# yeyupiaoling/VoiceprintRecognition-PaddlePaddle

Measured on AMD Instinct MI355X. Metric: utterances/sec (3 s, 16 kHz) ECAPA-TDNN fwd+AAM, higher is better.
Workload: dtype bf16; 1 GPU; BASELINE configs[1]: ECAPA-TDNN (C=512, MFA 1536, ASP, embd 192) + Kaldi Fbank 80, 3 s @ 16 kHz (T=298), 2796-class cosine head + AAMLoss, eval-mode forward, batch 256 per GPU, inputs resident in HBM, random-init weights; batch_per_gpu=256, global_batch=256, parallelism=dp1 (no collective), streams_per_gpu=2, hip_graph=True, graph_prereplays=40

## Files before the change

include/vpmi.h:

```cpp
#ifndef VPMI_H
#define VPMI_H
#include <stddef.h>
#include <stdint.h>

#ifdef __cplusplus
extern "C" {
#endif

#define VPMI_VERSION 100

typedef struct vp_ctx vp_ctx;
typedef void* vp_stream;

enum { VP_OK = 0, VP_EINVAL = -1, VP_ENOMEM = -2, VP_EHIP = -3, VP_EUNSUP = -4, VP_EWORKSPACE = -5 };
enum { VP_F32 = 0, VP_BF16 = 1,
       VP_F32X3 = 2,
       VP_HL32 = 3 };
enum { VP_PAD_NONE = 0, VP_PAD_REFLECT = 1, VP_PAD_ZERO = 2 };
enum { VP_ACT_NONE = 0, VP_ACT_RELU = 1, VP_ACT_SIGMOID = 2, VP_ACT_TANH = 3,
       VP_ACT_HARDTANH20 = 4,
       VP_ACT_SILU = 5 };

int vp_version(void);
vp_ctx* vp_create(int device);
void vp_destroy(vp_ctx* ctx);
const char* vp_last_error(vp_ctx* ctx);
int vp_set_margin_table(vp_ctx* ctx, const float* table);

typedef struct {
    int sample_rate;
    int n_mels;
    float frame_length_ms;
    float frame_shift_ms;
    float preemph;
    int remove_dc;
    float low_freq;
    float high_freq;
    float log_floor;
} vp_fbank_opts;

void vp_fbank_default_opts(vp_fbank_opts* o);
int vp_fbank_num_frames(const vp_fbank_opts* o, int n_samples);
size_t vp_fbank_workspace_bytes(const vp_fbank_opts* o, int B, int L);
int vp_fbank_cmn_f32(vp_ctx* ctx, const float* wav, const float* lens_ratio, int B, int L,
                     const vp_fbank_opts* o, float* out, void* out_bf16, void* ws, size_t ws_bytes,
                     vp_stream stream);
int vp_fbank_cmn_pcm16(vp_ctx* ctx, const int16_t* wav, float pcm_scale, const float* lens_ratio, int B, int L,
                       const vp_fbank_opts* o, float* out, void* out_bf16, void* ws, size_t ws_bytes, vp_stream stream);

int vp_fbank_cmn_ragged_f32(vp_ctx* ctx, const float* wav, const int32_t* n_samples, int B, int L, const vp_fbank_opts* o,
                            float* out, void* out_bf16, int32_t* n_frames, void* ws, size_t ws_bytes, vp_stream stream);

typedef struct {
    int sample_rate;
    int n_fft;
    int hop_length;
    int win_length;
    int n_mels;
    float f_min;
    float f_max;
    float power;
    int log_db;
    float amin;
    float ref_value;
} vp_mel_opts;

void vp_mel_default_opts(vp_mel_opts* o);
int vp_mel_num_frames(const vp_mel_opts* o, int n_samples);
size_t vp_mel_workspace_bytes(const vp_mel_opts* o, int B, int L);
int vp_melspec_cmn_f32(vp_ctx* ctx, const float* wav, const float* lens_ratio, int B, int L,
                       const vp_mel_opts* o, float* out, void* out_bf16, void* ws, size_t ws_bytes,
                       vp_stream stream);

int vp_melspec_cmn_ragged_f32(vp_ctx* ctx, const float* wav, const int32_t* n_samples, int B, int L, const vp_mel_opts* o,
                              float* out, void* out_bf16, int32_t* n_frames, void* ws, size_t ws_bytes, vp_stream stream);

typedef struct {
    int dtype_in, dtype_out;
    int B, T_in, T_out;
    int Cin, Cout, KW, dilation, stride, pad_left, pad_mode;
    const void* x;   int ldx, xoff;
    const void* w;
    const float* bias;
    const float* rowbias;
    int act;
    const float* bn_scale;
    const float* bn_shift;
    int act2;
    void* y;         int ldy, yoff;
    void* y2;        int ldy2, y2off, ysplit;
    const void* add_in; int ld_add, add_off;
    void* aux;       int ld_aux, aux_off;
    float* psum;
    float* psumsq;
    int F_in, F_out, KF, stride_f, pad_f;
    const float* pro_scale;
    const float* pro_shift;
    const void* res; int ld_res, res_off;
    const float* gate; int gate_len, gate_nseg;
    int mfma_bf16;
} vp_conv1d_desc;

int vp_conv1d_tiles_m(int B, int T_out);
int vp_conv1d_nseg(int T_out);
int vp_conv1d_fwd(vp_ctx* ctx, const vp_conv1d_desc* d, vp_stream stream);
enum { VP_CONV_K128 = 0,
       VP_CONV_K256_TWO_STAGE = 1,
       VP_CONV_K256_RING = 2,
       VP_CONV_K128X256_RING = 3 };
int vp_conv1d_plan(const vp_conv1d_desc* d, int* kernel, int* tile_n, int* tiles_m, int* tiles_n, int* group_m, int* launches);
int vp_conv256_select(int schedule);

int vp_moments_finalize(vp_ctx* ctx, const float* psum, const float* psumsq, const float* shift,
                        int B, int T, int C, float eps, int want_std, float* stats, vp_stream stream);
int vp_moments_finalize_affine(vp_ctx* ctx, const float* psum, const float* psumsq, const float* scale, const float* shift,
                               int B, int T, int C, float eps, int want_std, float* stats, vp_stream stream);

int vp_dense_f32(vp_ctx* ctx, const float* a, int lda, const float* w, int w_is_kn, const float* bias,
                 int M, int N, int K, int act, float* out, int ldo, vp_stream stream);

int vp_cast_f32_bf16(vp_ctx* ctx, const float* x, void* y, long long n, vp_stream stream);


int vp_se_scale_residual(vp_ctx* ctx, int dtype, const void* x, int ldx, int xoff, const float* s,
                         const void* res, int ldr, int roff, void* out, int ldo, int ooff,
                         int B, int T, int C, vp_stream stream);
int vp_se_scale_residual_shadow(vp_ctx* ctx, const float* x, int ldx, int xoff, const float* s, const float* res, int ldr, int roff,
                                float* out, int ldo, int ooff, void* shadow, int ld_shadow, int shadow_off, int B, int T, int C,
                                vp_stream stream);

int vp_asp_softmax_stats(vp_ctx* ctx, int dtype, const float* logits, const void* x, int ldx, int xoff,
                         int B, int T, int C, float eps, float* pooled, vp_stream stream);

#define VP_MAX_SE_BLOCKS 8
#define VP_MAX_RES2 15

typedef struct {
    const void* w;
    const float* bias;
    const float* bn_scale;
    const float* bn_shift;
    int cin, cout, kw, dil;
    const void* w_hl;
} vp_tdnn_layer;

typedef struct {
    vp_tdnn_layer tdnn1;
    vp_tdnn_layer res2[VP_MAX_RES2];
    vp_tdnn_layer tdnn2;
    const float* se_w1;
    const float* se_b1;
    const float* se_w2;
    const float* se_b2;
} vp_se_res2_block;

typedef struct {
    vp_tdnn_layer tdnn;
    const float* w_ctx;
    const void* conv_w;
    const float* conv_b;
    int C, att;
} vp_asp_weights;

typedef struct {
    int dtype;
    int feat_dim, embd_dim, n_blocks, res2_scale, se_ch;
    vp_tdnn_layer block0;
    vp_se_res2_block blk[VP_MAX_SE_BLOCKS];
    vp_tdnn_layer mfa;
    vp_asp_weights asp;
    const float* fc_w;
    const float* fc_b;
} vp_ecapa_weights;

int vp_res2_chain_fwd(vp_ctx* ctx, const vp_tdnn_layer* layers, int nconv, const void* t1, void* r2, int B, int T, int C,
                      int width, vp_stream stream);
int vp_asp_fused_fwd(vp_ctx* ctx, const void* h, const void* w, const float* bias, const void* x, int ldx, const float* center,
                     int ldc, int B, int T, int C, int att, float eps, float* pooled, vp_stream stream);
int vp_se_gate_fwd(vp_ctx* ctx, const float* psum, const float* shift, int B, int T, int C, int H, const float* w1, const float* b1,
                   const float* w2, const float* b2, float* out, vp_stream stream);
int vp_asp_utt_fwd(vp_ctx* ctx, const void* x, int ldx, const vp_tdnn_layer* tdnn, const float* rowbias, const void* conv_w,
                   const float* conv_b, int B, int T, int C, int att, float eps, float* pooled, vp_stream stream);

int vp_res2_chain_x3_fwd(vp_ctx* ctx, const vp_tdnn_layer* layers, int nconv, const void* t1, void* r2, int B, int T, int C,
                         int width, vp_stream stream);
int vp_res2_chain_x3_plan(int T, int nconv, int dil, int* nsplit, int* tseg, int* tp, int* lds_bytes);
int vp_ecapa_x3_fast_path(const vp_ecapa_weights* w, int B, int T);
int vp_asp_fused_x3_fwd(vp_ctx* ctx, const void* h, const float* w, const float* bias, const void* x, int ldx, const float* center,
                        int ldc, int B, int T, int C, int att, float eps, float* pooled, vp_stream stream);

size_t vp_ecapa_workspace_bytes(const vp_ecapa_weights* w, int B, int T);
int vp_ecapa_fwd(vp_ctx* ctx, const vp_ecapa_weights* w, const void* feats, int B, int T, float* emb,
                 void* ws, size_t ws_bytes, vp_stream stream);

typedef struct {
    int dtype;
    int feat_dim, embd_dim, channels;
    vp_tdnn_layer td[5];
    vp_asp_weights asp;
    const float* lin_w;
    const float* lin_b;
} vp_tdnn_weights;

size_t vp_tdnn_workspace_bytes(const vp_tdnn_weights* w, int B, int T);
int vp_tdnn_fwd(vp_ctx* ctx, const vp_tdnn_weights* w, const void* feats, int B, int T, float* emb,
                void* ws, size_t ws_bytes, vp_stream stream);

#define VP_MAX_CAM_LAYERS 64
#define VP_MAX_CAM_BLOCKS 4

typedef struct {
    vp_tdnn_layer conv1, conv2, shortcut;
    int stride, has_shortcut;
} vp_resblock;

typedef struct {
    const float* bn1_scale;
    const float* bn1_shift;
    vp_tdnn_layer linear1;
    vp_tdnn_layer local;
    const float* ctx_w1;
    const float* ctx_b1;
    const float* ctx_w2;
    const float* ctx_b2;
} vp_cam_layer;

typedef struct {
    const float* bn_scale;
    const float* bn_shift;
    vp_tdnn_layer linear;
} vp_transit;

typedef struct {
    int dtype;
    int feat_dim, embd_dim, m_channels, init_channels, growth, bn_channels, seg_len;
    int n_blocks;
    int block_layers[VP_MAX_CAM_BLOCKS];
    const float* fcm1_w;
    const float* fcm1_b;
    const float* fcm1_scale;
    const float* fcm1_shift;
    vp_resblock res[4];
    vp_tdnn_layer fcm_conv2;
    vp_tdnn_layer tdnn;
    vp_cam_layer layers[VP_MAX_CAM_LAYERS];
    vp_transit transit[VP_MAX_CAM_BLOCKS];
    const float* out_bn_scale;
    const float* out_bn_shift;
    const float* dense_w;
    const float* dense_b;
} vp_campplus_weights;

int vp_cam_block_fwd(vp_ctx* ctx, const vp_cam_layer* layers, int n_layers, void* cat, int ld, int ch0, int B, int Tn, int seg_len,
                     int bn_channels, int growth, vp_stream stream);
int vp_resblock_c32_fwd(vp_ctx* ctx, const void* x, void* y, const vp_tdnn_layer* conv1, const vp_tdnn_layer* conv2, int B, int T, int F,
                        vp_stream stream);
int vp_conv3x3_c32_fwd(vp_ctx* ctx, const void* x, void* y, const vp_tdnn_layer* conv, const void* res, int relu,
                       const vp_tdnn_layer* shortcut, void* y2, int B, int T, int F_in, int stride_f, const void* c1_feats,
                       const float* c1_w, const float* c1_b, const float* c1_scale, const float* c1_shift, vp_stream stream);

size_t vp_campplus_workspace_bytes(const vp_campplus_weights* w, int B, int T);
int vp_campplus_fwd(vp_ctx* ctx, const vp_campplus_weights* w, const void* feats, int B, int T, float* emb,
                    void* ws, size_t ws_bytes, vp_stream stream);

int vp_spec_augment(vp_ctx* ctx, int dtype, void* feats, int B, int T, int F, const int32_t* fmask, int n_freq_masks,
                    const int32_t* tmask, int n_time_masks, int replace_with_zero, vp_stream stream);
int vp_pad_batch(vp_ctx* ctx, int dtype, const void* const* srcs, const int32_t* lens, int B, int Tmax, int F, void* out,
                 vp_stream stream);
int vp_wave_batch_f32(vp_ctx* ctx, const float* const* srcs, const int32_t* lens, const int32_t* starts, int B, int L,
                      int normalize, float target_db, const float* gain_db, float* out, int32_t* n_valid, vp_stream stream);
int vp_speed_perturb_f32(vp_ctx* ctx, const float* const* srcs, const int32_t* lens, const int32_t* new_lens,
                         float* const* dsts, int B, int max_new_len, vp_stream stream);
int vp_noise_mix_f32(vp_ctx* ctx, const float* const* srcs, const int32_t* lens, const float* const* noises,
                     const int32_t* noise_lens, const int32_t* noise_starts, const float* snr_db, float* const* dsts, int B,
                     vp_stream stream);
size_t vp_reverb_workspace_bytes(int B, int max_len, int max_rir_len);
int vp_reverb_f32(vp_ctx* ctx, const float* const* srcs, const int32_t* lens, const float* const* rirs, const int32_t* rir_lens,
                  float* const* dsts, int B, int max_len, int max_rir_len, void* ws, size_t ws_bytes, vp_stream stream);

#define VP_MAX_RSE_BLOCKS 32

typedef struct {
    vp_tdnn_layer conv1, conv2, conv3, down;
    const float* se_w1;
    const float* se_b1;
    const float* se_w2;
    const float* se_b2;
    int stride, has_down;
} vp_rse_block;

typedef struct {
    int dtype;
    int feat_dim, embd_dim, n_blocks, c1_channels;
    const float* c1_w;
    const float* c1_b;
    const float* c1_scale;
    const float* c1_shift;
    vp_rse_block blk[VP_MAX_RSE_BLOCKS];
    vp_asp_weights asp;
    const float* lin_w;
    const float* lin_b;
} vp_resnetse_weights;

int vp_pointwise_fwd(vp_ctx* ctx, const vp_conv1d_desc* d, vp_stream stream);
size_t vp_resnetse_workspace_bytes(const vp_resnetse_weights* w, int B, int T);
int vp_resnetse_fwd(vp_ctx* ctx, const vp_resnetse_weights* w, const void* feats, int B, int T, float* emb,
                    void* ws, size_t ws_bytes, vp_stream stream);

#define VP_MAX_ERE_BLOCKS 40
#define VP_MAX_ERE_SCALE 4

typedef struct { vp_tdnn_layer c1, c2; } vp_aff_weights;

typedef struct {
    vp_tdnn_layer conv1;
    vp_tdnn_layer convs[VP_MAX_ERE_SCALE];
    vp_tdnn_layer conv3;
    vp_tdnn_layer shortcut;
    vp_aff_weights fuse[VP_MAX_ERE_SCALE - 1];
    int stride, has_shortcut, use_aff, width, scale;
} vp_ere_block;

typedef struct {
    int dtype;
    int feat_dim, embd_dim, n_blocks, m_channels;
    int stage_blocks[4];
    int first_fuse;
    const float* c1_w;
    const float* c1_b;
    const float* c1_scale;
    const float* c1_shift;
    vp_ere_block blk[VP_MAX_ERE_BLOCKS];
    vp_tdnn_layer down[3];
    vp_aff_weights fuse[3];
    const float* seg_w;
    const float* seg_b;
} vp_eres2net_weights;

size_t vp_eres2net_workspace_bytes(const vp_eres2net_weights* w, int B, int T);
int vp_eres2net_fwd(vp_ctx* ctx, const vp_eres2net_weights* w, const void* feats, int B, int T, float* emb,
                    void* ws, size_t ws_bytes, vp_stream stream);

#define VP_MAX_R2N_BLOCKS 32
#define VP_MAX_R2N_SCALE 8

typedef struct {
    vp_tdnn_layer conv1;
    vp_tdnn_layer convs[VP_MAX_R2N_SCALE];
    vp_tdnn_layer conv3;
    vp_tdnn_layer down;
    int stride, has_down, stage, width, scale;
} vp_r2n_block;

typedef struct {
    int dtype;
    int feat_dim, embd_dim, n_blocks, m_channels;
    const float* c1_w;
    const float* c1_b;
    const float* c1_scale;
    const float* c1_shift;
    vp_r2n_block blk[VP_MAX_R2N_BLOCKS];
    vp_asp_weights asp;
    const float* lin_w;
    const float* lin_b;
} vp_res2net_weights;

size_t vp_res2net_workspace_bytes(const vp_res2net_weights* w, int B, int T);
int vp_res2net_fwd(vp_ctx* ctx, const vp_res2net_weights* w, const void* feats, int B, int T, float* emb,
                   void* ws, size_t ws_bytes, vp_stream stream);
int vp_res2net_stem_fwd(vp_ctx* ctx, int dtype, const void* feats, void* out, const float* w, const float* bias, const float* scale,
                        const float* shift, int B, int T, int F, int C, vp_stream stream);
int vp_avgpool3x3_fwd(vp_ctx* ctx, int dtype, const void* x, int ldx, int xoff, void* y, int ldy, int yoff, int B, int T, int F, int C,
                      int stride, vp_stream stream);
int vp_avgpool3x3_bwd_f32(vp_ctx* ctx, const float* dy, int lddy, int dyoff, float* dx, int lddx, int dxoff, int B, int T, int F, int C,
                          int stride, vp_stream stream);
int vp_maxpool3x3_fwd_f32(vp_ctx* ctx, const float* x, float* y, int B, int T, int F, int C, vp_stream stream);
int vp_maxpool3x3_bwd_f32(vp_ctx* ctx, const float* x, const float* dy, float* dx, int B, int T, int F, int C, vp_stream stream);

size_t vp_cosine_logits_workspace_bytes(int B, int D, int C);
int vp_cosine_logits_f32(vp_ctx* ctx, const float* emb, const float* W, int B, int D, int C, float* logits,
                         void* ws, size_t ws_bytes, vp_stream stream);
int vp_aam_ce_fwd(vp_ctx* ctx, const float* logits, const int64_t* labels, int B, int C, float margin, float scale,
                  float label_smoothing, int easy_margin, float* loss, float* row_loss,
                  vp_stream stream);
size_t vp_cosine_aam_workspace_bytes(int B, int D, int C);
int vp_cosine_aam_ce_fwd(vp_ctx* ctx, const float* emb, const float* W, const int64_t* labels, int B, int D,
                         int C, float margin, float scale, float label_smoothing, int easy_margin,
                         float* loss, float* logits, float* row_loss, void* ws, size_t ws_bytes,
                         vp_stream stream);

size_t vp_cosine_aam_tiled_workspace_bytes(int B, int D, int C);
int vp_cosine_aam_tiled_fwd(vp_ctx* ctx, const float* emb, const float* W, const int64_t* labels, int B, int D, int C, float margin,
                            float scale, float label_smoothing, int easy_margin, float* loss, float* row_loss, float* lse,
                            float* cinv, int* pred, void* ws, size_t ws_bytes, vp_stream stream);

size_t vp_cosine_aam_tiled_bwd_workspace_bytes(int B, int D, int C);
int vp_cosine_aam_tiled_bwd(vp_ctx* ctx, const float* emb, const float* W, const int64_t* labels, int B, int D, int C, float margin,
                            float scale, float label_smoothing, int easy_margin, float grad_scale, float* demb, float* dW, float* loss,
                            int* pred, void* ws, size_t ws_bytes, vp_stream stream);

size_t vp_cosine_aam_ce_bwd_workspace_bytes(int B, int D, int C);
int vp_cosine_aam_ce_bwd(vp_ctx* ctx, const float* emb, const float* W, const int64_t* labels, int B, int D, int C, float margin,
                         float scale, float label_smoothing, int easy_margin, float grad_scale, float* demb, float* dW,
                         float* loss, void* ws, size_t ws_bytes, vp_stream stream);

int vp_aam_ce_bwd(vp_ctx* ctx, const float* logits, const int64_t* labels, int B, int C, float margin, float scale,
                  float label_smoothing, int easy_margin, float grad_scale, float* dlogits, float* loss, float* row_loss,
                  vp_stream stream);
size_t vp_cosine_logits_bwd_workspace_bytes(int B, int D, int C);
int vp_cosine_logits_bwd(vp_ctx* ctx, const float* emb, const float* W, const float* dcos, int B, int D, int C, float* demb,
                         float* dW, void* ws, size_t ws_bytes, vp_stream stream);

enum { VP_LOSS_AAM = 0, VP_LOSS_AM = 1, VP_LOSS_ARM = 2, VP_LOSS_CE = 3, VP_LOSS_SUBCENTER = 4 };
int vp_margin_ce_fwd(vp_ctx* ctx, const float* logits, const int64_t* labels, int B, int C, int K, int kind, float margin,
                     float scale, float label_smoothing, int easy_margin, float* loss, float* row_loss, vp_stream stream);
int vp_margin_ce_bwd(vp_ctx* ctx, const float* logits, const int64_t* labels, int B, int C, int K, int kind, float margin,
                     float scale, float label_smoothing, int easy_margin, float grad_scale, float* dlogits, float* loss,
                     float* row_loss, vp_stream stream);
int vp_sphereface2(vp_ctx* ctx, const float* logits, const int64_t* labels, const float* bias, int B, int C, float margin,
                   float scale, float lanbuda, int t, int margin_type_a, float grad_scale, float* loss, float* row_loss,
                   float* dlogits, float* dbias, float* row_dbias, vp_stream stream);

size_t vp_conv1d_wgrad_workspace_bytes(const vp_conv1d_desc* d);
int vp_conv1d_wgrad_f32(vp_ctx* ctx, const vp_conv1d_desc* d, const float* dz, int lddz, float* dW, void* ws, size_t ws_bytes,
                        vp_stream stream);
int vp_conv1d_wgrad_oik_f32(vp_ctx* ctx, const vp_conv1d_desc* d, const float* dz, int lddz, float* dW, void* ws, size_t ws_bytes,
                            vp_stream stream);
int vp_conv_weight_layouts_f32(vp_ctx* ctx, const float* w, int Cout, int Cin, int KW, float* wp, float* w2, vp_stream stream);
int vp_conv2d_weight_layouts_f32(vp_ctx* ctx, const float* w, int Cout, int Cin, int KF, int KT, float* wp, float* w2, vp_stream stream);
int vp_prep_weights_bf16(vp_ctx* ctx, const void* const* w, void* const* w16, void* const* wt16, const int* rows, const int* cols,
                         const int* ld, int n, vp_stream stream);
size_t vp_col_sums_workspace_bytes(long long M, int C);
int vp_col_sums_f32(vp_ctx* ctx, const float* a, int lda, const float* b, int ldb, const float* bmean, const float* bscale,
                    long long M, int C, float* sums, void* ws, size_t ws_bytes, vp_stream stream);
int vp_bn_train_finalize(vp_ctx* ctx, const float* psum, const float* psumsq, int nparts, long long M, int C, const float* gamma,
                         const float* beta, float* running_mean, float* running_var, float momentum, float eps, float* mean,
                         float* invstd, float* scale, float* shift, vp_stream stream);
int vp_affine_rows_f32(vp_ctx* ctx, const float* z, int ldz, const float* scale, const float* shift, long long M, int C, float* y,
                       int ldy, int relu, vp_stream stream);
int vp_bn_relu_bwd_f32(vp_ctx* ctx, const float* dy, int lddy, const float* z, int ldz, const float* mean, const float* invstd,
                       const float* gamma, const float* sums, long long M, int C, int relu_mask, float* dz, int lddz,
                       vp_stream stream);
size_t vp_bn_relu_bwd_dbias_workspace_bytes(long long M, int C);
int vp_bn_relu_bwd_dbias_f32(vp_ctx* ctx, const float* dy, int lddy, const float* z, int ldz, const float* mean, const float* invstd,
                             const float* gamma, const float* sums, long long M, int C, int relu_mask, float* dz, int lddz,
                             float* dbias, void* ws, size_t ws_bytes, vp_stream stream);
int vp_bn_relu_bwd_dbias_bf16out(vp_ctx* ctx, const float* dy, int lddy, const float* z, int ldz, const float* mean, const float* invstd,
                                 const float* gamma, const float* sums, long long M, int C, int relu_mask, void* dz, int lddz,
                                 float* dbias, void* ws, size_t ws_bytes, vp_stream stream);
int vp_conv1d_wgrad_bf16_oik(vp_ctx* ctx, const vp_conv1d_desc* d, const void* dz, int lddz, float* dW, void* ws, size_t ws_bytes,
                             vp_stream stream);
int vp_affine_rows_b16_f32(vp_ctx* ctx, const void* z, int ldz, const float* scale, const float* shift, long long M, int C, float* y,
                           int ldy, int relu, vp_stream stream);
int vp_col_sums_f32_b16(vp_ctx* ctx, const float* a, int lda, const void* b, int ldb, const float* bmean, const float* bscale, long long M,
                        int C, float* sums, void* ws, size_t ws_bytes, vp_stream stream);
int vp_bn_relu_bwd_dbias_b16(vp_ctx* ctx, const float* dy, int lddy, const void* z, int ldz, const float* mean, const float* invstd,
                             const float* gamma, const float* sums, long long M, int C, int relu_mask, void* dz, int lddz,
                             float* dbias, void* ws, size_t ws_bytes, vp_stream stream);
int vp_pack_segments_f32(vp_ctx* ctx, const void* const* srcs, const long long* offs, const long long* sizes, int n, float* dst,
                         vp_stream stream);
int vp_adam_step_f32(vp_ctx* ctx, float* param, const float* grad, float* m, float* v, long long n, float lr, float beta1, float beta2,
                     float eps, float weight_decay, int step, float grad_scale, vp_stream stream);
int vp_adamw_step_f32(vp_ctx* ctx, float* param, const float* grad, float* m, float* v, long long n, float lr, float beta1, float beta2,
                      float eps, float coeff, int step, float grad_scale, vp_stream stream);
int vp_momentum_step_f32(vp_ctx* ctx, float* param, const float* grad, float* velocity, long long n, float lr, float momentum,
                         float weight_decay, int use_nesterov, float grad_scale, vp_stream stream);

int vp_utt_sums_f32(vp_ctx* ctx, const float* a, int lda, int B, int T, int C, float* out, vp_stream stream);
int vp_time_stats_f32(vp_ctx* ctx, const float* x, int ldx, int B, int T, int C, float eps, int unbiased ,
                      float* stats, vp_stream stream);
int vp_time_stats_bwd_add_f32(vp_ctx* ctx, const float* x, int ldx, const float* stats, const float* dstats, int B, int T, int C, float eps,
                              int unbiased, const float* add, int ldadd, float* dx, int lddx, vp_stream stream);
int vp_time_stats_bwd_f32(vp_ctx* ctx, const float* x, int ldx, const float* stats, const float* dstats, int B, int T, int C, float eps,
                          int unbiased, float* dx, int lddx, vp_stream stream);
int vp_attn_stats_bwd_f32(vp_ctx* ctx, const float* e, const float* x, int ldx, const float* pooled, const float* dpooled, int B, int T,
                          int C, float eps, float* de, float* dx, int lddx, vp_stream stream);
int vp_attn_stats_bwd_de16(vp_ctx* ctx, const float* e, const float* x, int ldx, const float* pooled, const float* dpooled, int B, int T,
                           int C, float eps, void* de, float* dx, int lddx, vp_stream stream);
int vp_asp_softmax_stats_l16(vp_ctx* ctx, const void* logits_bf16, const void* x, int x_dtype, int ldx, int xoff, int B, int T, int C, float eps,
// ... 123 lines not shown
```

voiceprintrecognition-paddlepaddle_amd/csrc/res2_chain.hip:

```cpp
#include "common.h"

namespace {

constexpr int R2_W = 64;
constexpr int R2_K = 3 * R2_W;
constexpr int R2_THREADS = 512;
constexpr int R2_WAVES = R2_THREADS / 64;
constexpr int R2_ROUNDS = 3;
typedef __attribute__((address_space(3))) void* r2_lds_ptr;

struct Res2Args {
    const bf16_t* t1;
    bf16_t* r2;
    const bf16_t* w[VP_MAX_RES2];
    const float* bias[VP_MAX_RES2];
    const float* scale[VP_MAX_RES2];
    const float* shift[VP_MAX_RES2];
    int T, C, nconv, dil, TP;
    unsigned t1_bytes;
#ifdef VP_TIMING
    unsigned long long* dbg;
#endif
};

__device__ __forceinline__ int reflect_idx(int t, int T) {
    t = t < 0 ? -t : t;
    return t >= T ? 2 * (T - 1) - t : t;
}

__global__ __launch_bounds__(R2_THREADS, 1) void res2_chain_kernel(Res2Args a) {
    extern __shared__ __attribute__((aligned(16))) char smem[];
    const int act_bytes = a.TP * 128;
    char* act0 = smem;
    char* wt0 = smem + 2 * act_bytes;
    constexpr int WT_BYTES = R2_W * R2_K * 2;
#ifdef VP_TIMING
    unsigned long long stamps[32];
    int nst = 0;
    stamps[nst++] = wall_clock64();
#endif
    const int tid = threadIdx.x, lane = tid & 63;
    const int wv = __builtin_amdgcn_readfirstlane(tid >> 6);
    const int li = lane & 15, g = lane >> 4;
    const int b = blockIdx.x;
    const size_t row0 = (size_t)b * a.T;
    constexpr unsigned OOB = 0xfffffff0u;
    const __amdgpu_buffer_rsrc_t xsrd = __builtin_amdgcn_make_buffer_rsrc(const_cast<bf16_t*>(a.t1), 0, a.t1_bytes, 0x00020000);

    const int drow = lane >> 3;
    const unsigned dchunk = (unsigned)((lane & 7) ^ drow) << 4;
    auto dma_x = [&](int slice, char* dst) {
        const unsigned colb = (unsigned)slice * (R2_W * 2) + dchunk;
        for (int p = wv; p < a.TP / 8; p += R2_WAVES) {
            const int t = p * 8 + drow;
            const unsigned off = t < a.T ? (unsigned)((row0 + t) * a.C * 2) + colb : OOB;
            __builtin_amdgcn_raw_ptr_buffer_load_lds(xsrd, (r2_lds_ptr)(dst + p * 1024), 16, off, 0, 0, 0);
        }
    };
    auto dma_w = [&](int j, char* dst) {
        const __amdgpu_buffer_rsrc_t wsrd = __builtin_amdgcn_make_buffer_rsrc(const_cast<bf16_t*>(a.w[j]), 0, WT_BYTES, 0x00020000);
#pragma unroll
        for (int u = 0; u < 3; ++u) {
            const int p = wv + u * R2_WAVES;
            const int tap = p >> 3, nb = (p & 7) * 8;
            const unsigned off = (unsigned)((nb + drow) * (R2_K * 2) + tap * 128) + dchunk;
            __builtin_amdgcn_raw_ptr_buffer_load_lds(wsrd, (r2_lds_ptr)(dst + tap * 8192 + nb * 128), 16, off, 0, 0, 0);
        }
    };

    dma_x(1, act0);
    dma_w(0, wt0);
    const int ntile = a.TP / 16;
    float* prm = reinterpret_cast<float*>(wt0 + 2 * WT_BYTES);
    for (int i = tid; i < a.nconv * 192; i += R2_THREADS) {
        const int j = i / 192, k = i - j * 192, which = k >> 6, n = k & 63;
        prm[i] = which == 0 ? a.bias[j][n] : (which == 1 ? a.scale[j][n] : a.shift[j][n]);
    }
    asm volatile("s_waitcnt vmcnt(0)" ::: "memory");
    __syncthreads();
#ifdef VP_TIMING
    stamps[nst++] = wall_clock64();
#endif

    for (int j = 0; j < a.nconv; ++j) {
        char* ain = act0 + (j & 1) * act_bytes;
        char* aout = act0 + ((j + 1) & 1) * act_bytes;
        const char* wl = wt0 + (j & 1) * WT_BYTES;
        const bool has_next = j + 1 < a.nconv;
        if (has_next) {
            dma_x(j + 2, aout);
            dma_w(j + 1, wt0 + ((j + 1) & 1) * WT_BYTES);
        }
        bf16x8 wf[4][6];
#pragma unroll
        for (int ni = 0; ni < 4; ++ni) {
            const int n = ni * 16 + li;
#pragma unroll
            for (int s = 0; s < 6; ++s) {
                const int c = (s & 1) * 4 + g;
                wf[ni][s] = *reinterpret_cast<const bf16x8*>(wl + (s >> 1) * 8192 + n * 128 + ((c ^ (n & 7)) << 4));
            }
        }
        f32x4 acc[R2_ROUNDS][4];
#pragma unroll
        for (int r = 0; r < R2_ROUNDS; ++r) {
            const int mt = wv + r * R2_WAVES;
            const int t = min(mt * 16 + li, a.TP - 1);
#pragma unroll
            for (int ni = 0; ni < 4; ++ni) acc[r][ni] = f32x4{0.f, 0.f, 0.f, 0.f};
#pragma unroll
            for (int tap = 0; tap < 3; ++tap) {
                int ts = reflect_idx(t + (tap - 1) * a.dil, a.T);
                ts = min(max(ts, 0), a.TP - 1);
#pragma unroll
                for (int ks = 0; ks < 2; ++ks) {
                    const int c = ks * 4 + g;
                    const bf16x8 xf = *reinterpret_cast<const bf16x8*>(ain + ts * 128 + ((c ^ (ts & 7)) << 4));
#pragma unroll
                    for (int ni = 0; ni < 4; ++ni)
                        acc[r][ni] = __builtin_amdgcn_mfma_f32_16x16x32_bf16(wf[ni][tap * 2 + ks], xf, acc[r][ni], 0, 0, 0);
                }
            }
        }
#ifdef VP_TIMING
        if (nst < 32) stamps[nst++] = wall_clock64();
#endif
        asm volatile("s_waitcnt vmcnt(0)" ::: "memory");
        __syncthreads();
#ifdef VP_TIMING
        if (nst < 32) stamps[nst++] = wall_clock64();
#endif
        const float* pj = prm + j * 192;
#pragma unroll
        for (int r = 0; r < R2_ROUNDS; ++r) {
            const int mt = wv + r * R2_WAVES;
            if (mt < ntile) {
                const int t = mt * 16 + li;
#pragma unroll
                for (int ni = 0; ni < 4; ++ni) {
                    const int nb = ni * 16 + g * 4;
                    const float4 bb = *reinterpret_cast<const float4*>(pj + nb);
                    const float4 ss = *reinterpret_cast<const float4*>(pj + 64 + nb);
                    const float4 hh = *reinterpret_cast<const float4*>(pj + 128 + nb);
                    float v[4];
                    v[0] = fmaxf(acc[r][ni][0] + bb.x, 0.f) * ss.x + hh.x;
                    v[1] = fmaxf(acc[r][ni][1] + bb.y, 0.f) * ss.y + hh.y;
                    v[2] = fmaxf(acc[r][ni][2] + bb.z, 0.f) * ss.z + hh.z;
                    v[3] = fmaxf(acc[r][ni][3] + bb.w, 0.f) * ss.w + hh.w;
                    const int pos = t * 128 + (((nb >> 3) ^ (t & 7)) << 4) + (nb & 7) * 2;
                    bf16x4 o;
                    o[0] = (bf16_t)v[0]; o[1] = (bf16_t)v[1]; o[2] = (bf16_t)v[2]; o[3] = (bf16_t)v[3];
                    *reinterpret_cast<bf16x4*>(ain + pos) = o;
                    if (has_next) {
                        const bf16x4 xn = *reinterpret_cast<const bf16x4*>(aout + pos);
                        bf16x4 s;
                        s[0] = (bf16_t)(v[0] + (float)xn[0]); s[1] = (bf16_t)(v[1] + (float)xn[1]);
                        s[2] = (bf16_t)(v[2] + (float)xn[2]); s[3] = (bf16_t)(v[3] + (float)xn[3]);
                        *reinterpret_cast<bf16x4*>(aout + pos) = s;
                    }
                }
            }
        }
        __syncthreads();
#ifdef VP_TIMING
        if (nst < 32) stamps[nst++] = wall_clock64();
#endif
        {
            bf16_t* ybase = a.r2 + row0 * a.C + (j + 1) * R2_W;
            for (int i = tid; i < a.T * 8; i += R2_THREADS) {
                const int t = i >> 3, c = i & 7;
                const uint4 v = *reinterpret_cast<const uint4*>(ain + t * 128 + ((c ^ (t & 7)) << 4));
                *reinterpret_cast<uint4*>(ybase + (size_t)t * a.C + c * 8) = v;
            }
        }
        __syncthreads();
#ifdef VP_TIMING
        if (nst < 32) stamps[nst++] = wall_clock64();
#endif
    }
#ifdef VP_TIMING
    if (a.dbg && tid == 0)
        for (int i = 0; i < 32; ++i) a.dbg[(size_t)b * 32 + i] = i < nst ? stamps[i] : 0;
#endif
}

}

#ifdef VP_TIMING
static unsigned long long* g_res2_dbg = nullptr;
extern "C" void vp_dbg_res2_buffer(void* p) { g_res2_dbg = (unsigned long long*)p; }
#endif

int vp_res2_chain_bf16(vp_ctx* ctx, const vp_tdnn_layer* layers, int nconv, const void* t1, void* r2, int B, int T,
                       int C, int width, hipStream_t st) {
    if (width != R2_W || nconv < 1 || nconv > VP_MAX_RES2) return VP_EUNSUP;
    const int TP = (T + 15) / 16 * 16;
    const size_t smem = (size_t)2 * TP * 128 + 2 * (size_t)R2_W * R2_K * 2 + (size_t)nconv * 192 * 4;
    if (smem > 160 * 1024 || T < 2 || TP / 16 > R2_WAVES * R2_ROUNDS) return VP_EUNSUP;
    const int dil = layers[0].dil;
    Res2Args a;
    memset(&a, 0, sizeof(a));
    for (int j = 0; j < nconv; ++j) {
        const vp_tdnn_layer& L = layers[j];
        if (L.kw != 3 || L.cin != R2_W || L.cout != R2_W || L.dil != dil || !L.bias || !L.bn_scale || !L.bn_shift)
            return VP_EUNSUP;
        a.w[j] = (const bf16_t*)L.w; a.bias[j] = L.bias; a.scale[j] = L.bn_scale; a.shift[j] = L.bn_shift;
    }
    if (dil >= T) return VP_EUNSUP;
    a.t1 = (const bf16_t*)t1; a.r2 = (bf16_t*)r2; a.T = T; a.C = C; a.nconv = nconv; a.dil = dil; a.TP = TP;
    const unsigned long long t1b = (unsigned long long)B * T * C * 2;
    if (t1b >= 0xffffff00ull || (C * 2) % 16 || (reinterpret_cast<uintptr_t>(t1) | reinterpret_cast<uintptr_t>(r2)) & 15) return VP_EUNSUP;
    a.t1_bytes = (unsigned)t1b;
#ifdef VP_TIMING
    a.dbg = g_res2_dbg;
#endif
    static bool attr_dev[64] = {};
    bool& attr_set = attr_dev[ctx->device & 63];
    if (!attr_set) {
        VP_HIP(ctx, hipFuncSetAttribute(reinterpret_cast<const void*>(res2_chain_kernel),
                                        hipFuncAttributeMaxDynamicSharedMemorySize, 160 * 1024));
        attr_set = true;
    }
    hipLaunchKernelGGL(res2_chain_kernel, dim3(B), dim3(R2_THREADS), smem, st, a);
    VP_LAUNCH_CHECK(ctx, "res2_chain");
    return VP_OK;
}
```

voiceprintrecognition-paddlepaddle_amd/ppvector/_abi.py:

```python
import ctypes as C
import re
from types import SimpleNamespace

SCALARS = {'int': C.c_int, 'int32_t': C.c_int, 'float': C.c_float, 'size_t': C.c_size_t, 'long long': C.c_longlong}
POINTEES = {'void', 'char', 'float', 'int', 'int16_t', 'int32_t', 'int64_t', 'long long'}
TYPE = r'(?:const\s+)?(long long|\w+)\s*((?:\*\s*(?:const\s*)?)*)'


class AbiError(ValueError):
    pass


def parse(text, class_names):
    consts, structs, protos = {}, {}, {}
    scalars, pointees = dict(SCALARS), set(POINTEES)

    def ctype(base, stars, what, ret=False):
        n = stars.count('*')
        if n == 0 and base in scalars:
            return scalars[base]
        if n == 0 and base in structs and not ret:
            return structs[base]
        if n and base in pointees:
            return C.c_char_p if ret and base == 'char' and n == 1 else C.c_void_p
        if n == 1 and base in structs:
            return C.POINTER(structs[base])
        raise AbiError(f'vpmi.h: no ctypes type for "{base}{stars.strip()}" in "{what}"')

    def bound(expr, what):
        m = re.fullmatch(r'(\w+)(?:\s*-\s*(\d+))?', expr.strip())
        head = m and (int(m[1]) if m[1].isdigit() else consts.get(m[1]))
        if head is None:
            raise AbiError(f'vpmi.h: array bound "{expr}" in "{what}" is neither a literal nor a known constant')
        return head - int(m[2] or 0)

    def enum(body):
        for item in filter(None, (i.strip() for i in body.split(','))):
            m = re.fullmatch(r'(\w+)\s*=\s*(-?\d+)', item)
            if not m:
                raise AbiError(f'vpmi.h: enumerator "{item}" is not NAME = <int>')
            consts[m[1]] = int(m[2])

    def struct(body, name):
        if name not in class_names:
            raise AbiError(f'vpmi.h: struct {name} has no Python class name')
        fields = []
        for decl in filter(None, (d.strip() for d in body.split(';'))):
            m = re.match(TYPE, decl)
            names = decl[m.end():].split(',') if m else []
            if not names or m[2] and len(names) > 1:
                raise AbiError(f'vpmi.h: cannot read the field "{decl}" of {name}')
            t = ctype(m[1], m[2], decl)
            for d in names:
                f = re.fullmatch(r'\s*(\w+)\s*(?:\[([^\]]+)\])?\s*', d)
                if not f:
                    raise AbiError(f'vpmi.h: cannot read the field "{decl}" of {name}')
                fields.append((f[1], t * bound(f[2], decl) if f[2] else t))
        structs[name] = type(class_names[name], (C.Structure,), {'_fields_': fields})

    def function(ret, stars, name, args):
        what = f'{name}({" ".join(args.split())})'
        argtypes = []
        for a in ([] if args.strip() == 'void' else args.split(',')):
            m = re.fullmatch(r'\s*' + TYPE + r'\w+\s*', a)
            if not m:
                raise AbiError(f'vpmi.h: cannot read the parameter "{a.strip()}" of {name}')
            argtypes.append(ctype(m[1], m[2], what))
        protos[name] = (None if (ret, stars) == ('void', '') else ctype(ret, stars, what, ret=True), argtypes)

    def declaration(dname, dvalue, ebody, sbody, sname, ret, stars, fname, args):
        if dname:
            consts[dname] = int(dvalue)
        elif ebody is not None:
            enum(ebody)
        elif sname:
            struct(sbody, sname)
        else:
            function(ret, stars, fname, args)
        return ''

    text = re.sub(r'/\*.*?\*/', ' ', text, flags=re.S)
    text = re.sub(r'^[ \t]*#[ \t]*(ifndef \w+|ifdef \w+|define \w+|include <[\w.]+>|endif)[ \t]*$', '', text, flags=re.M)
    text = re.sub(r'\A\s*extern "C" \{(.*)\}\s*\Z', r'\1', text, flags=re.S)
    text = re.sub(r'\btypedef struct (\w+) \1;', lambda m: pointees.add(m[1]) or '', text)
    text = re.sub(r'\btypedef void\s*\* (\w+);', lambda m: scalars.update({m[1]: C.c_void_p}) or '', text)
    text = re.sub(r'^[ \t]*#[ \t]*define[ \t]+(\w+)[ \t]+(-?\d+)[ \t]*$'
                  r'|\benum \{([^{}]*)\};'
                  r'|\btypedef struct \{([^{}]*)\}\s*(\w+);'
                  r'|^\s*' + TYPE + r'(\w+)\s*\(([^(){};]*)\)\s*;', lambda m: declaration(*m.groups()), text, flags=re.M)
    if text.strip():
        raise AbiError(f'vpmi.h: cannot read "{" ".join(text.split())[:120]}"')
    return SimpleNamespace(consts=consts, structs=structs, protos=protos)
```

Before: 203,300 utterances/s.

## Pipeline Res2 chain with triple activation buffer and async copy-out

```diff
diff --git a/include/vpmi.h b/include/vpmi.h
--- a/include/vpmi.h
+++ b/include/vpmi.h
@@ -175,6 +175,8 @@
 
 int vp_res2_chain_fwd(vp_ctx* ctx, const vp_tdnn_layer* layers, int nconv, const void* t1, void* r2, int B, int T, int C,
                       int width, vp_stream stream);
+enum { VP_RES2_TWO_BUFFER = 0, VP_RES2_PIPELINED = 1 };
+int vp_res2_chain_plan(int T, int nconv, int dil, int* schedule, size_t* lds_bytes);
 int vp_asp_fused_fwd(vp_ctx* ctx, const void* h, const void* w, const float* bias, const void* x, int ldx, const float* center,
                      int ldc, int B, int T, int C, int att, float eps, float* pooled, vp_stream stream);
 int vp_se_gate_fwd(vp_ctx* ctx, const float* psum, const float* shift, int B, int T, int C, int H, const float* w1, const float* b1,
diff --git a/voiceprintrecognition-paddlepaddle_amd/csrc/res2_chain.hip b/voiceprintrecognition-paddlepaddle_amd/csrc/res2_chain.hip
--- a/voiceprintrecognition-paddlepaddle_amd/csrc/res2_chain.hip
+++ b/voiceprintrecognition-paddlepaddle_amd/csrc/res2_chain.hip
@@ -1,4 +1,11 @@
 #include "common.h"
+
+#ifndef R2_NH
+#define R2_NH 2
+#endif
+#ifndef R2_PF
+#define R2_PF 1
+#endif
 
 namespace {
 
@@ -7,7 +14,14 @@
 constexpr int R2_THREADS = 512;
 constexpr int R2_WAVES = R2_THREADS / 64;
 constexpr int R2_ROUNDS = 3;
+constexpr int R2_WT_BYTES = R2_W * R2_K * 2;
+constexpr int R2_LDS_MAX = 160 * 1024;
+constexpr int R2_NT = 4 / R2_NH;
+constexpr int R2_NR = R2_ROUNDS * R2_NH;
+constexpr int R2_TSTEP = R2_WAVES / R2_NH;
+constexpr int R2_CO = R2_ROUNDS * R2_WAVES * 16 * 8 / R2_THREADS;
 typedef __attribute__((address_space(3))) void* r2_lds_ptr;
+typedef __attribute__((ext_vector_type(4))) unsigned u32x4;
 
 struct Res2Args {
     const bf16_t* t1;
@@ -23,17 +37,52 @@
 #endif
 };
 
+struct Res2Plan { int TP, schedule; size_t lds; };
+
+bool res2_plan(int T, int nconv, int dil, Res2Plan& p) {
+    p = Res2Plan{0, 0, 0};
+    if (nconv < 1 || nconv > VP_MAX_RES2 || T < 2 || dil >= T) return false;
+    const int TP = (T + 15) / 16 * 16;
+    if (TP / 16 > R2_WAVES * R2_ROUNDS) return false;
+    const size_t fixed = (size_t)R2_WT_BYTES + (size_t)nconv * 192 * 4;
+    const size_t lds3 = (size_t)3 * TP * 128 + fixed;
+    p.TP = TP;
+#ifdef R2_FORCE_TWO_BUFFER
+    p.schedule = VP_RES2_TWO_BUFFER;
+#else
+    p.schedule = lds3 <= R2_LDS_MAX ? VP_RES2_PIPELINED : VP_RES2_TWO_BUFFER;
+#endif
+    p.lds = p.schedule == VP_RES2_PIPELINED ? lds3 : (size_t)2 * TP * 128 + fixed;
+    return p.lds <= R2_LDS_MAX;
+}
+
+__device__ __forceinline__ void r2_dma16(u32x4 rsrc, unsigned lds_addr, unsigned voff) {
+    lds_addr = __builtin_amdgcn_readfirstlane(lds_addr);
+    rsrc = u32x4{(unsigned)__builtin_amdgcn_readfirstlane(rsrc[0]), (unsigned)__builtin_amdgcn_readfirstlane(rsrc[1]),
+                 (unsigned)__builtin_amdgcn_readfirstlane(rsrc[2]), (unsigned)__builtin_amdgcn_readfirstlane(rsrc[3])};
+    asm volatile("s_mov_b32 m0, %0\n\ts_nop 0\n\tbuffer_load_dwordx4 %1, %2, 0 offen lds"
+                 :: "s"(lds_addr), "v"(voff), "s"(rsrc) : "memory");
+}
+__device__ __forceinline__ u32x4 r2_rsrc(const void* p, unsigned bytes) {
+    const unsigned long long q = reinterpret_cast<unsigned long long>(p);
+    return u32x4{(unsigned)q, (unsigned)(q >> 32) & 0xffffu, bytes, 0x00020000u};
+}
+__device__ __forceinline__ unsigned r2_lds_addr(const char* p) {
+    return (unsigned)reinterpret_cast<uintptr_t>((r2_lds_ptr)(const_cast<char*>(p)));
+}
+
 __device__ __forceinline__ int reflect_idx(int t, int T) {
     t = t < 0 ? -t : t;
     return t >= T ? 2 * (T - 1) - t : t;
 }
 
+template <bool PIPE>
 __global__ __launch_bounds__(R2_THREADS, 1) void res2_chain_kernel(Res2Args a) {
     extern __shared__ __attribute__((aligned(16))) char smem[];
+    constexpr int NACT = PIPE ? 3 : 2;
     const int act_bytes = a.TP * 128;
     char* act0 = smem;
-    char* wt0 = smem + 2 * act_bytes;
-    constexpr int WT_BYTES = R2_W * R2_K * 2;
+    char* wt0 = smem + NACT * act_bytes;
 #ifdef VP_TIMING
     unsigned long long stamps[32];
     int nst = 0;
@@ -45,7 +94,8 @@
     const int b = blockIdx.x;
     const size_t row0 = (size_t)b * a.T;
     constexpr unsigned OOB = 0xfffffff0u;
-    const __amdgpu_buffer_rsrc_t xsrd = __builtin_amdgcn_make_buffer_rsrc(const_cast<bf16_t*>(a.t1), 0, a.t1_bytes, 0x00020000);
+    const u32x4 xsrd = r2_rsrc(a.t1, a.t1_bytes);
+    const __amdgpu_buffer_rsrc_t ysrd = __builtin_amdgcn_make_buffer_rsrc(a.r2, 0, a.t1_bytes, 0x00020000);
 
     const int drow = lane >> 3;
     const unsigned dchunk = (unsigned)((lane & 7) ^ drow) << 4;
@@ -54,131 +104,232 @@
         for (int p = wv; p < a.TP / 8; p += R2_WAVES) {
             const int t = p * 8 + drow;
             const unsigned off = t < a.T ? (unsigned)((row0 + t) * a.C * 2) + colb : OOB;
-            __builtin_amdgcn_raw_ptr_buffer_load_lds(xsrd, (r2_lds_ptr)(dst + p * 1024), 16, off, 0, 0, 0);
-        }
-    };
-    auto dma_w = [&](int j, char* dst) {
-        const __amdgpu_buffer_rsrc_t wsrd = __builtin_amdgcn_make_buffer_rsrc(const_cast<bf16_t*>(a.w[j]), 0, WT_BYTES, 0x00020000);
+            r2_dma16(xsrd, r2_lds_addr(dst + p * 1024), off);
+        }
+    };
+    auto dma_w = [&](int j) {
+        const u32x4 wsrd = r2_rsrc(a.w[j], R2_WT_BYTES);
 #pragma unroll
         for (int u = 0; u < 3; ++u) {
             const int p = wv + u * R2_WAVES;
             const int tap = p >> 3, nb = (p & 7) * 8;
             const unsigned off = (unsigned)((nb + drow) * (R2_K * 2) + tap * 128) + dchunk;
-            __builtin_amdgcn_raw_ptr_buffer_load_lds(wsrd, (r2_lds_ptr)(dst + tap * 8192 + nb * 128), 16, off, 0, 0, 0);
-        }
-    };
-
+            r2_dma16(wsrd, r2_lds_addr(wt0 + tap * 8192 + nb * 128), off);
+        }
+    };
+    const int npiece = wv < a.TP / 8 ? (a.TP / 8 - 1 - wv) / R2_WAVES + 1 : 0;
+    auto co_read = [&](u32x4 (&v)[R2_CO], const char* src) {
+        const char* s0 = src + (wv * 8 + drow) * 128 + (((lane & 7) ^ drow) << 4);
+#pragma unroll
+        for (int k = 0; k < R2_CO; ++k) {
+            v[k] = u32x4{0u, 0u, 0u, 0u};
+            if (k < npiece) v[k] = *reinterpret_cast<const u32x4*>(s0 + k * R2_WAVES * 1024);
+        }
+    };
+    auto co_store = [&](const u32x4 (&v)[R2_CO], int slice) {
+        unsigned off0 = (unsigned)(((row0 + wv * 8 + drow) * a.C + (lane & 7) * 8) * 2);
+        asm volatile("" : "+v"(off0));
+        const int step = R2_WAVES * 8 * a.C * 2;
+#pragma unroll
+        for (int k = 0; k < R2_CO; ++k) {
+            const int t = (wv + k * R2_WAVES) * 8 + drow;
+            __builtin_amdgcn_raw_buffer_store_b128(v[k], ysrd, t < a.T ? off0 : OOB, k * step + slice * (R2_W * 2), 0);
+        }
+    };
+    auto wait_vm = [&](int n) {
+        switch (n) {
+            case 1: asm volatile("s_waitcnt vmcnt(1)" ::: "memory"); break;
+            case 2: asm volatile("s_waitcnt vmcnt(2)" ::: "memory"); break;
+            case 3: asm volatile("s_waitcnt vmcnt(3)" ::: "memory"); break;
+            case 4: asm volatile("s_waitcnt vmcnt(4)" ::: "memory"); break;
+            case 5: asm volatile("s_waitcnt vmcnt(5)" ::: "memory"); break;
+            case 6: asm volatile("s_waitcnt vmcnt(6)" ::: "memory"); break;
+            case 7: asm volatile("s_waitcnt vmcnt(7)" ::: "memory"); break;
+            case 8: asm volatile("s_waitcnt vmcnt(8)" ::: "memory"); break;
+            case 9: asm volatile("s_waitcnt vmcnt(9)" ::: "memory"); break;
+            case 10: asm volatile("s_waitcnt vmcnt(10)" ::: "memory"); break;
+            case 11: asm volatile("s_waitcnt vmcnt(11)" ::: "memory"); break;
+            case 12: asm volatile("s_waitcnt vmcnt(12)" ::: "memory"); break;
+            default: asm volatile("s_waitcnt vmcnt(0)" ::: "memory"); break;
+        }
+    };
+    auto barrier = [&]() {
+        asm volatile("s_waitcnt lgkmcnt(0)" ::: "memory");
+        __builtin_amdgcn_s_barrier();
+        asm volatile("" ::: "memory");
+    };
+
+    const int ntile = a.TP / 16;
+    const int tile0 = wv / R2_NH, nbase = (wv % R2_NH) * (R2_W / R2_NH);
+    const int nr = tile0 < ntile ? (ntile - 1 - tile0) / R2_TSTEP + 1 : 0;
+    bf16x8 wf[R2_NT][6];
+    auto load_wf = [&]() {
+#pragma unroll
+        for (int ni = 0; ni < R2_NT; ++ni) {
+            const int n = nbase + ni * 16 + li;
+#pragma unroll
+            for (int s = 0; s < 6; ++s) {
+                const int c = (s & 1) * 4 + g;
+                wf[ni][s] = *reinterpret_cast<const bf16x8*>(wt0 + (s >> 1) * 8192 + n * 128 + ((c ^ (n & 7)) << 4));
+            }
+        }
+    };
+    int xo[R2_NR][3];
+#pragma unroll
+    for (int r = 0; r < R2_NR; ++r) {
+        const int t = min((tile0 + r * R2_TSTEP) * 16 + li, a.TP - 1);
+#pragma unroll
+        for (int tap = 0; tap < 3; ++tap) {
+            int ts = reflect_idx(t + (tap - 1) * a.dil, a.T);
+            ts = min(max(ts, 0), a.TP - 1);
+            xo[r][tap] = ts * 128 + ((g ^ (ts & 7)) << 4);
+        }
+    }
+
+    float* prm = reinterpret_cast<float*>(wt0 + R2_WT_BYTES);
+    for (int j = wv; j < a.nconv; j += R2_WAVES) {
+        const float pb = a.bias[j][lane], ps = a.scale[j][lane], ph = a.shift[j][lane];
+        prm[j * 192 + lane] = pb; prm[j * 192 + 64 + lane] = ps; prm[j * 192 + 128 + lane] = ph;
+    }
     dma_x(1, act0);
-    dma_w(0, wt0);
-    const int ntile = a.TP / 16;
-    float* prm = reinterpret_cast<float*>(wt0 + 2 * WT_BYTES);
-    for (int i = tid; i < a.nconv * 192; i += R2_THREADS) {
-        const int j = i / 192, k = i - j * 192, which = k >> 6, n = k & 63;
-        prm[i] = which == 0 ? a.bias[j][n] : (which == 1 ? a.scale[j][n] : a.shift[j][n]);
-    }
+    if (PIPE && a.nconv > 1) dma_x(2, act0 + act_bytes);
+    dma_w(0);
     asm volatile("s_waitcnt vmcnt(0)" ::: "memory");
     __syncthreads();
+    load_wf();
+    __syncthreads();
 #ifdef VP_TIMING
     stamps[nst++] = wall_clock64();
 #endif
 
     for (int j = 0; j < a.nconv; ++j) {
-        char* ain = act0 + (j & 1) * act_bytes;
-        char* aout = act0 + ((j + 1) & 1) * act_bytes;
-        const char* wl = wt0 + (j & 1) * WT_BYTES;
+        char* ain = act0 + (j % NACT) * act_bytes;
+        char* aout = act0 + ((j + 1) % NACT) * act_bytes;
+        char* aprev = act0 + ((j + NACT - 1) % NACT) * act_bytes;
         const bool has_next = j + 1 < a.nconv;
-        if (has_next) {
-            dma_x(j + 2, aout);
-            dma_w(j + 1, wt0 + ((j + 1) & 1) * WT_BYTES);
-        }
-        bf16x8 wf[4][6];
-#pragma unroll
-        for (int ni = 0; ni < 4; ++ni) {
-            const int n = ni * 16 + li;
-#pragma unroll
-            for (int s = 0; s < 6; ++s) {
-                const int c = (s & 1) * 4 + g;
-                wf[ni][s] = *reinterpret_cast<const bf16x8*>(wl + (s >> 1) * 8192 + n * 128 + ((c ^ (n & 7)) << 4));
-            }
-        }
-        f32x4 acc[R2_ROUNDS][4];
-#pragma unroll
-        for (int r = 0; r < R2_ROUNDS; ++r) {
-            const int mt = wv + r * R2_WAVES;
-            const int t = min(mt * 16 + li, a.TP - 1);
-#pragma unroll
-            for (int ni = 0; ni < 4; ++ni) acc[r][ni] = f32x4{0.f, 0.f, 0.f, 0.f};
-#pragma unroll
-            for (int tap = 0; tap < 3; ++tap) {
-                int ts = reflect_idx(t + (tap - 1) * a.dil, a.T);
-                ts = min(max(ts, 0), a.TP - 1);
-#pragma unroll
-                for (int ks = 0; ks < 2; ++ks) {
-                    const int c = ks * 4 + g;
-                    const bf16x8 xf = *reinterpret_cast<const bf16x8*>(ain + ts * 128 + ((c ^ (ts & 7)) << 4));
-#pragma unroll
-                    for (int ni = 0; ni < 4; ++ni)
-                        acc[r][ni] = __builtin_amdgcn_mfma_f32_16x16x32_bf16(wf[ni][tap * 2 + ks], xf, acc[r][ni], 0, 0, 0);
-                }
+        const bool more_x = j + NACT <= a.nconv;
+        int in_flight = 0;
+        {
+            u32x4 yv[R2_CO];
+            if (j > 0) {
+                co_read(yv, aprev);
+                asm volatile("s_waitcnt lgkmcnt(0)" ::: "memory");
+            }
+            if (has_next) dma_w(j + 1);
+            if (more_x) {
+                dma_x(j + NACT, aprev);
+                if (PIPE) in_flight += npiece;
+            }
+            if (j > 0) {
+                co_store(yv, j);
+                in_flight += R2_CO;
             }
         }
 #ifdef VP_TIMING
         if (nst < 32) stamps[nst++] = wall_clock64();
 #endif
-        asm volatile("s_waitcnt vmcnt(0)" ::: "memory");
-        __syncthreads();
+        f32x4 acc[R2_NR][R2_NT];
+        bf16x8 xf[6];
+        auto load_x = [&](int r, int s) {
+            xf[s] = *reinterpret_cast<const bf16x8*>(ain + (xo[r][s >> 1] ^ ((s & 1) * 64)));
+        };
+        if (R2_PF) {
+#pragma unroll
+            for (int s = 0; s < 6; ++s) load_x(0, s);
+        }
+#pragma unroll
+        for (int r = 0; r < R2_NR; ++r) {
+#pragma unroll
+            for (int ni = 0; ni < R2_NT; ++ni) acc[r][ni] = f32x4{0.f, 0.f, 0.f, 0.f};
+            if (r < nr) {
+                if (!R2_PF) {
+#pragma unroll
+                    for (int s = 0; s < 6; ++s) load_x(r, s);
+                }
+#pragma unroll
+                for (int s = 0; s < 6; ++s) {
+#pragma unroll
+                    for (int ni = 0; ni < R2_NT; ++ni)
+                        acc[r][ni] = __builtin_amdgcn_mfma_f32_16x16x32_bf16(wf[ni][s], xf[s], acc[r][ni], 0, 0, 0);
+                    if (R2_PF && r + 1 < R2_NR) load_x(r + 1, s);
+                }
+                if (R2_PF && r + 1 < R2_NR) {
+#pragma unroll
+                    for (int s = 0; s < 6; ++s) {
+                        __builtin_amdgcn_sched_group_barrier(0x008, R2_NT, 0);
+                        __builtin_amdgcn_sched_group_barrier(0x100, 1, 0);
+                    }
+                }
+            }
+        }
 #ifdef VP_TIMING
         if (nst < 32) stamps[nst++] = wall_clock64();
 #endif
+        wait_vm(in_flight);
+        barrier();
+#ifdef VP_TIMING
+        if (nst < 32) stamps[nst++] = wall_clock64();
+#endif
         const float* pj = prm + j * 192;
-#pragma unroll
-        for (int r = 0; r < R2_ROUNDS; ++r) {
-            const int mt = wv + r * R2_WAVES;
-            if (mt < ntile) {
-                const int t = mt * 16 + li;
-#pragma unroll
-                for (int ni = 0; ni < 4; ++ni) {
-                    const int nb = ni * 16 + g * 4;
-                    const float4 bb = *reinterpret_cast<const float4*>(pj + nb);
-                    const float4 ss = *reinterpret_cast<const float4*>(pj + 64 + nb);
-                    const float4 hh = *reinterpret_cast<const float4*>(pj + 128 + nb);
+        float4 bb[R2_NT], ss[R2_NT], hh[R2_NT];
+#pragma unroll
+        for (int ni = 0; ni < R2_NT; ++ni) {
+            const int nb = nbase + ni * 16 + g * 4;
+            bb[ni] = *reinterpret_cast<const float4*>(pj + nb);
+            ss[ni] = *reinterpret_cast<const float4*>(pj + 64 + nb);
+            hh[ni] = *reinterpret_cast<const float4*>(pj + 128 + nb);
+        }
+        bf16x4 xn[R2_NR][R2_NT];
+#pragma unroll
+        for (int r = 0; r < R2_NR; ++r) {
+            if (has_next && r < nr) {
+                const int t = (tile0 + r * R2_TSTEP) * 16 + li;
+#pragma unroll
+                for (int ni = 0; ni < R2_NT; ++ni) {
+                    const int nb = nbase + ni * 16 + g * 4;
+                    xn[r][ni] = *reinterpret_cast<const bf16x4*>(aout + t * 128 + (((nb >> 3) ^ (t & 7)) << 4) + (nb & 7) * 2);
+                }
+            }
+        }
+#pragma unroll
+        for (int r = 0; r < R2_NR; ++r) {
+            if (r < nr) {
+                const int t = (tile0 + r * R2_TSTEP) * 16 + li;
+#pragma unroll
+                for (int ni = 0; ni < R2_NT; ++ni) {
+                    const int nb = nbase + ni * 16 + g * 4;
                     float v[4];
-                    v[0] = fmaxf(acc[r][ni][0] + bb.x, 0.f) * ss.x + hh.x;
-                    v[1] = fmaxf(acc[r][ni][1] + bb.y, 0.f) * ss.y + hh.y;
-                    v[2] = fmaxf(acc[r][ni][2] + bb.z, 0.f) * ss.z + hh.z;
-                    v[3] = fmaxf(acc[r][ni][3] + bb.w, 0.f) * ss.w + hh.w;
+                    v[0] = fmaxf(acc[r][ni][0] + bb[ni].x, 0.f) * ss[ni].x + hh[ni].x;
+                    v[1] = fmaxf(acc[r][ni][1] + bb[ni].y, 0.f) * ss[ni].y + hh[ni].y;
+                    v[2] = fmaxf(acc[r][ni][2] + bb[ni].z, 0.f) * ss[ni].z + hh[ni].z;
+                    v[3] = fmaxf(acc[r][ni][3] + bb[ni].w, 0.f) * ss[ni].w + hh[ni].w;
                     const int pos = t * 128 + (((nb >> 3) ^ (t & 7)) << 4) + (nb & 7) * 2;
                     bf16x4 o;
                     o[0] = (bf16_t)v[0]; o[1] = (bf16_t)v[1]; o[2] = (bf16_t)v[2]; o[3] = (bf16_t)v[3];
                     *reinterpret_cast<bf16x4*>(ain + pos) = o;
                     if (has_next) {
-                        const bf16x4 xn = *reinterpret_cast<const bf16x4*>(aout + pos);
                         bf16x4 s;
-                        s[0] = (bf16_t)(v[0] + (float)xn[0]); s[1] = (bf16_t)(v[1] + (float)xn[1]);
-                        s[2] = (bf16_t)(v[2] + (float)xn[2]); s[3] = (bf16_t)(v[3] + (float)xn[3]);
+                        s[0] = (bf16_t)(v[0] + (float)xn[r][ni][0]); s[1] = (bf16_t)(v[1] + (float)xn[r][ni][1]);
+                        s[2] = (bf16_t)(v[2] + (float)xn[r][ni][2]); s[3] = (bf16_t)(v[3] + (float)xn[r][ni][3]);
                         *reinterpret_cast<bf16x4*>(aout + pos) = s;
                     }
                 }
             }
         }
-        __syncthreads();
+        __builtin_amdgcn_sched_barrier(0);
+        load_wf();
+        barrier();
 #ifdef VP_TIMING
         if (nst < 32) stamps[nst++] = wall_clock64();
 #endif
-        {
-            bf16_t* ybase = a.r2 + row0 * a.C + (j + 1) * R2_W;
-            for (int i = tid; i < a.T * 8; i += R2_THREADS) {
-                const int t = i >> 3, c = i & 7;
-                const uint4 v = *reinterpret_cast<const uint4*>(ain + t * 128 + ((c ^ (t & 7)) << 4));
-                *reinterpret_cast<uint4*>(ybase + (size_t)t * a.C + c * 8) = v;
-            }
-        }
-        __syncthreads();
-#ifdef VP_TIMING
-        if (nst < 32) stamps[nst++] = wall_clock64();
-#endif
-    }
-#ifdef VP_TIMING
+    }
+    {
+        u32x4 yv[R2_CO];
+        co_read(yv, act0 + ((a.nconv - 1) % NACT) * act_bytes);
+        co_store(yv, a.nconv);
+    }
+#ifdef VP_TIMING
+    if (nst < 32) stamps[nst++] = wall_clock64();
     if (a.dbg && tid == 0)
         for (int i = 0; i < 32; ++i) a.dbg[(size_t)b * 32 + i] = i < nst ? stamps[i] : 0;
 #endif
@@ -194,10 +345,9 @@
 int vp_res2_chain_bf16(vp_ctx* ctx, const vp_tdnn_layer* layers, int nconv, const void* t1, void* r2, int B, int T,
                        int C, int width, hipStream_t st) {
     if (width != R2_W || nconv < 1 || nconv > VP_MAX_RES2) return VP_EUNSUP;
-    const int TP = (T + 15) / 16 * 16;
-    const size_t smem = (size_t)2 * TP * 128 + 2 * (size_t)R2_W * R2_K * 2 + (size_t)nconv * 192 * 4;
-    if (smem > 160 * 1024 || T < 2 || TP / 16 > R2_WAVES * R2_ROUNDS) return VP_EUNSUP;
     const int dil = layers[0].dil;
+    Res2Plan p;
+    if (!res2_plan(T, nconv, dil, p)) return VP_EUNSUP;
     Res2Args a;
     memset(&a, 0, sizeof(a));
     for (int j = 0; j < nconv; ++j) {
@@ -206,8 +356,7 @@
             return VP_EUNSUP;
         a.w[j] = (const bf16_t*)L.w; a.bias[j] = L.bias; a.scale[j] = L.bn_scale; a.shift[j] = L.bn_shift;
     }
-    if (dil >= T) return VP_EUNSUP;
-    a.t1 = (const bf16_t*)t1; a.r2 = (bf16_t*)r2; a.T = T; a.C = C; a.nconv = nconv; a.dil = dil; a.TP = TP;
+    a.t1 = (const bf16_t*)t1; a.r2 = (bf16_t*)r2; a.T = T; a.C = C; a.nconv = nconv; a.dil = dil; a.TP = p.TP;
     const unsigned long long t1b = (unsigned long long)B * T * C * 2;
     if (t1b >= 0xffffff00ull || (C * 2) % 16 || (reinterpret_cast<uintptr_t>(t1) | reinterpret_cast<uintptr_t>(r2)) & 15) return VP_EUNSUP;
     a.t1_bytes = (unsigned)t1b;
@@ -217,11 +366,22 @@
     static bool attr_dev[64] = {};
     bool& attr_set = attr_dev[ctx->device & 63];
     if (!attr_set) {
-        VP_HIP(ctx, hipFuncSetAttribute(reinterpret_cast<const void*>(res2_chain_kernel),
-                                        hipFuncAttributeMaxDynamicSharedMemorySize, 160 * 1024));
+        VP_HIP(ctx, hipFuncSetAttribute(reinterpret_cast<const void*>(res2_chain_kernel<true>),
+                                        hipFuncAttributeMaxDynamicSharedMemorySize, R2_LDS_MAX));
+        VP_HIP(ctx, hipFuncSetAttribute(reinterpret_cast<const void*>(res2_chain_kernel<false>),
+                                        hipFuncAttributeMaxDynamicSharedMemorySize, R2_LDS_MAX));
         attr_set = true;
     }
-    hipLaunchKernelGGL(res2_chain_kernel, dim3(B), dim3(R2_THREADS), smem, st, a);
+    if (p.schedule == VP_RES2_PIPELINED) hipLaunchKernelGGL(res2_chain_kernel<true>, dim3(B), dim3(R2_THREADS), p.lds, st, a);
+    else hipLaunchKernelGGL(res2_chain_kernel<false>, dim3(B), dim3(R2_THREADS), p.lds, st, a);
     VP_LAUNCH_CHECK(ctx, "res2_chain");
     return VP_OK;
 }
+
+extern "C" int vp_res2_chain_plan(int T, int nconv, int dil, int* schedule, size_t* lds_bytes) {
+    Res2Plan p;
+    const bool ok = res2_plan(T, nconv, dil, p);
+    if (schedule) *schedule = p.schedule;
+    if (lds_bytes) *lds_bytes = p.lds;
+    return ok ? VP_OK : VP_EUNSUP;
+}
diff --git a/voiceprintrecognition-paddlepaddle_amd/ppvector/_abi.py b/voiceprintrecognition-paddlepaddle_amd/ppvector/_abi.py
--- a/voiceprintrecognition-paddlepaddle_amd/ppvector/_abi.py
+++ b/voiceprintrecognition-paddlepaddle_amd/ppvector/_abi.py
@@ -3,7 +3,7 @@
 from types import SimpleNamespace
 
 SCALARS = {'int': C.c_int, 'int32_t': C.c_int, 'float': C.c_float, 'size_t': C.c_size_t, 'long long': C.c_longlong}
-POINTEES = {'void', 'char', 'float', 'int', 'int16_t', 'int32_t', 'int64_t', 'long long'}
+POINTEES = {'void', 'char', 'float', 'int', 'int16_t', 'int32_t', 'int64_t', 'long long', 'size_t'}
 TYPE = r'(?:const\s+)?(long long|\w+)\s*((?:\*\s*(?:const\s*)?)*)'
 
 
```

Result: no change. 204,500 utterances/s (median of 5 runs) (+0.6%).
